# louissmit/VBNN

Measured on NVIDIA B200. Metric: VB-MLP train samples/sec, higher is better.
Workload: dtype bf16

## Files before the change

### vbnn_b200/csrc/layer.cu

```cuda
#include <math.h>
#include <stdarg.h>
#include <string.h>

#include <vector>

#include "knobs.h"
#include "state.h"

namespace vbnn {

static thread_local char g_err[512] = "";

void set_error(const char* fmt, ...) {
  va_list ap;
  va_start(ap, fmt);
  vsnprintf(g_err, sizeof(g_err), fmt, ap);
  va_end(ap);
}

template <typename T>
static int dev_zalloc(T** p, size_t count, cudaStream_t st) {
  VB_TRY(dev_alloc(p, count));
  if (count) VB_CUDA(cudaMemsetAsync(*p, 0, count * sizeof(T), st));
  return VBNN_OK;
// ... 179 lines not shown
  int t = *reinterpret_cast<int*>(c->h_scalars) + 1;
  VB_CUDA(cudaMemcpyAsync(L->t_dev, &t, sizeof(int), cudaMemcpyHostToDevice, c->stream));
  VB_CUDA(cudaStreamSynchronize(c->stream));
  return VBNN_OK;
}

int layer_update_internal(vbnn_layer* L, vbnn_stats* stats, bool bump_t) {
  vbnn_ctx* c = L->ctx;
  cudaStream_t st = c->stream;
  const long long W = (long long)L->O * L->I;
  if (L->kind == VBNN_KIND_LINEAR) {
    VB_TRY(launch_sgd(L->weight, L->gW, W, &L->hp->lr_bias, L->w_bf16, L->I, L->ldI, st));
    VB_TRY(launch_sgd(L->bias, L->gb, L->O, &L->hp->lr_bias, nullptr, 1, 1, st));
    c->launches += 2;
    if (bump_t) VB_TRY(bump_layer_t(L));
    return VBNN_OK;
  }
  VB_TRY(launch_sgd(L->bias, L->gb, L->O, &L->hp->lr_bias, nullptr, 1, 1, st));
  UpdateParams u;
  memset(&u, 0, sizeof(u));
  u.mu = L->means; u.lvar = L->lvars; u.gW = L->gW; u.gS = L->gS;
  u.m_mu = L->m_mu; u.v_mu = L->v_mu; u.m_var = L->m_var; u.v_var = L->v_var;
  u.stdv = L->stdv; u.mu_sqe = L->mu_sqe;
  u.mu_bf16 = L->mu_bf16; u.s2_bf16 = L->s2_bf16; u.ld_bf16 = L->ldI; u.s2_f32 = L->s2_f32;
  u.O = L->O; u.I = L->I;
  u.partials = L->prior_partials; u.n_partials = L->n_part;
  u.next_partials = L->prior_partials; u.partials_pingpong = 1;
  u.var_hat_dev = L->var_hat_dev; u.t_dev = L->t_dev;
  u.S = (float)L->opts.S;
  u.hp = L->hp;
  u.lrt = layer_is_lrt(L);
  u.prior = layer_prior(L, 0);
  u.grid_override = L->n_part;
  u.coresident = knobs().upd_coresident != 0;
  double* stat_dev = stats ? c->d_partials + kMaxPartials : nullptr;
  u.stat_partials = stat_dev;
  int grid = 0;
  const double bytes = (L->prior_kind == VBNN_PRIOR_PER_WEIGHT ? 64.0 : 56.0) * (double)W;
  VB_TRY(prof_launch(c, 7, bytes, [&] { return launch_update(u, &grid, st); }));
  c->launches += 2;
  L->prior_valid = true;
  if (bump_t) VB_TRY(bump_layer_t(L));
  if (stats) {
    VB_CUDA(cudaMemcpyAsync(c->h_partials, stat_dev, (size_t)grid * kStatSlots * sizeof(double),
                            cudaMemcpyDeviceToHost, st));
    VB_CUDA(cudaMemcpyAsync(c->h_scalars, L->var_hat_dev, sizeof(float), cudaMemcpyDeviceToHost, st));
    VB_CUDA(cudaStreamSynchronize(st));
    double s[kStatSlots] = {0};
    s[11] = 3e38; s[12] = -3e38; s[13] = 3e38; s[14] = -3e38;
    for (int b = 0; b < grid; ++b) {
      const double* q = c->h_partials + (size_t)b * kStatSlots;
      for (int i = 0; i < 10; ++i) s[i] += q[i];
      s[11] = fmin(s[11], q[11]); s[12] = fmax(s[12], q[12]);
      s[13] = fmin(s[13], q[13]); s[14] = fmax(s[14], q[14]);
    }
    const double n = (double)W, nl = sqrt(s[4]), nm = sqrt(s[5]);
    stats->vlc_grad = (float)(sqrt(s[0]) / nl);
    stats->vle_grad = (float)(sqrt(s[1]) / nl);
    stats->mlc_grad = (float)(sqrt(s[2]) / nm);
    stats->mle_grad = (float)(sqrt(s[3]) / nm);
    stats->min_variance = (float)s[11];
    stats->max_variance = (float)s[12];
    stats->mean_variance = (float)(s[6] / n);
    stats->var_hat = c->h_scalars[0];
    const double mean = s[7] / n;
    stats->mean_means = (float)mean;
    stats->std_means = (float)sqrt(fmax(0.0, (s[5] - n * mean * mean) / (n - 1.0)));
    stats->min_means = (float)s[13];
    stats->max_means = (float)s[14];
    stats->mu_normratio = (float)(sqrt(s[8]) / nm);
    stats->var_normratio = (float)(sqrt(s[9]) / nl);
  }
  return VBNN_OK;
}

void weight_operands(GemmArgs& g, const vbnn_layer* L, int kmajor, bool batched, bool lrt) {
  const bool b16 = is_bf16(L), mu = layer_is_lrt(L);
  const int ld = b16 ? L->ldI : L->I;
  const void* w = b16 ? (mu ? (const void*)L->mu_bf16 : L->w_bf16) : (mu ? L->means : L->weight);
  g.B1 = {w, ld, kmajor, batched ? (long long)L->O * ld : 0};
  if (lrt) g.B2 = {b16 ? (const void*)L->s2_bf16 : L->s2_f32, ld, kmajor, 0};
}

int gemm(vbnn_ctx* c, bool bf16, int mode, const GemmArgs& g, const EpiParams& p, int prof_cls) {
  if (!bf16) return gemm_simt_launch(mode, g, p, c->stream, &c->launches);
  const int cls = (prof_cls >= 0 ? prof_cls : mode) & 7;
  const double flops = 2.0 * g.M * (double)g.N * g.K * g.batch * (epi_is_dual(mode) ? 2.0 : 1.0);
  return prof_launch(c, cls, flops, [&] { return gemm_tc_launch(mode, g, p, c->stream, &c->launches); });
}

int prof_mark(vbnn_ctx* c, int id) {
  if (!c->profiling) return VBNN_OK;
  cudaEvent_t e;
  if (!c->prof_pool.empty()) { e = c->prof_pool.back(); c->prof_pool.pop_back(); }
  else VB_CUDA(cudaEventCreate(&e));
  VB_CUDA(cudaEventRecord(e, c->stream));
  c->marks.push_back({e, id});
  return VBNN_OK;
}

int prof_collect(vbnn_ctx* c) {
  if (c->prof_recs.empty() && c->marks.empty()) return VBNN_OK;
  VB_CUDA(cudaStreamSynchronize(c->stream));
  for (size_t i = 0; i < c->marks.size(); ++i) {
    const int id = c->marks[i].id & 15;
    if (i > 0 && id != 0) {
      float ms = 0.f;
      VB_CUDA(cudaEventElapsedTime(&ms, c->marks[i - 1].e, c->marks[i].e));
      c->phase_ms[id] += ms; c->phase_n[id] += 1;
    }
  }
  for (auto& mk : c->marks) c->prof_pool.push_back(mk.e);
  c->marks.clear();
  for (auto& r : c->prof_recs) {
    float ms = 0.f;
    VB_CUDA(cudaEventElapsedTime(&ms, r.a, r.b));
    c->prof_ms[r.cls] += ms; c->prof_flops[r.cls] += r.flops; c->prof_n[r.cls] += 1;
    c->prof_pool.push_back(r.a); c->prof_pool.push_back(r.b);
  }
  c->prof_recs.clear();
  return VBNN_OK;
}

}

using namespace vbnn;

extern "C" int vbnn_abi_version(void) { return VBNN_ABI_VERSION; }
extern "C" const char* vbnn_last_error(void) { return g_err; }

extern "C" void vbnn_opts_default(vbnn_opts* o) {
  if (!o) return;
  memset(o, 0, sizeof(*o));
  o->var_init = 0.001f;
  o->msr_init = 0;
  o->mu_init = 0.f;
  o->B = 1000000.f;
  o->S = 30;
  o->lr_bias = 0.001f;
  o->lr_mu = 0.0001f;
  o->lr_var = 0.05f;
  o->adam_beta1 = 0.9f; o->adam_beta2 = 0.999f; o->adam_eps = 1e-8f;
  o->reparam = VBNN_REPARAM_WEIGHT;
  o->precision = VBNN_PREC_FP32;
  o->strict_reference = 1;
}

extern "C" int vbnn_ctx_create(int device, void* stream, uint64_t seed, vbnn_ctx** out) {
  return vbnn_ctx_create_ex(device, stream, VBNN_CTX_STREAM_GIVEN, seed, out);
}

extern "C" int vbnn_ctx_create_ex(int device, void* stream, int stream_mode, uint64_t seed, vbnn_ctx** out) {
  VB_CHECK(out != nullptr, VBNN_E_INVALID, "vbnn_ctx_create: out is null");
  VB_CHECK(stream_mode >= VBNN_CTX_STREAM_GIVEN && stream_mode <= VBNN_CTX_STREAM_PRIVATE_BLOCKING, VBNN_E_INVALID,
           "vbnn_ctx_create_ex: bad stream_mode %d", stream_mode);
  VB_CHECK(stream_mode == VBNN_CTX_STREAM_GIVEN || stream == nullptr, VBNN_E_INVALID,
           "vbnn_ctx_create_ex: stream must be NULL with stream_mode %d", stream_mode);
  int ndev = 0;
  cudaError_t e = cudaGetDeviceCount(&ndev);
  if (e != cudaSuccess || ndev == 0) {
    set_error("no CUDA device available (%s); libvbnn has no CPU fallback",
              e != cudaSuccess ? cudaGetErrorString(e) : "device count 0");
    return VBNN_E_CUDA;
  }
  VB_CHECK(device >= 0 && device < ndev, VBNN_E_INVALID, "vbnn_ctx_create: device %d of %d", device, ndev);
  VB_CUDA(cudaSetDevice(device));
  cudaDeviceProp prop;
  VB_CUDA(cudaGetDeviceProperties(&prop, device));
  VB_CHECK(prop.major == 10, VBNN_E_UNSUPPORTED,
           "libvbnn.so is built for sm_100a only; device %d is sm_%d%d", device, prop.major, prop.minor);
  vbnn_ctx* c = new vbnn_ctx();
  c->device = device; c->seed = seed;
  if (stream_mode == VBNN_CTX_STREAM_LEGACY_DEFAULT) {
    c->stream = cudaStreamLegacy;
    c->capturable = false;
  } else if (stream_mode == VBNN_CTX_STREAM_PRIVATE_BLOCKING) {
    VB_CUDA(cudaStreamCreateWithFlags(&c->stream, cudaStreamDefault));
    c->own_stream = true;
  } else if (stream) {
    c->stream = (cudaStream_t)stream;
    c->capturable = c->stream != cudaStreamLegacy && c->stream != cudaStreamPerThread;
  } else {
    VB_CUDA(cudaStreamCreateWithFlags(&c->stream, cudaStreamNonBlocking));
    c->own_stream = true;
  }
  VB_CUDA(cudaStreamCreateWithFlags(&c->copy_stream, cudaStreamNonBlocking));
  VB_TRY(dev_zalloc(&c->d_step, 1, c->stream));
  VB_TRY(dev_alloc(&c->d_partials, (size_t)kMaxPartials * (1 + kStatSlots)));
  VB_CUDA(cudaMallocHost((void**)&c->h_partials, (size_t)kMaxPartials * kStatSlots * sizeof(double)));
  VB_CUDA(cudaMallocHost((void**)&c->h_scalars, 4096 * sizeof(float)));
  *out = c;
  return VBNN_OK;
}

extern "C" int vbnn_ctx_destroy(vbnn_ctx* c) {
  if (!c) return VBNN_OK;
  cudaSetDevice(c->device);
  cudaStreamSynchronize(c->stream);
  prof_collect(c);
  for (cudaEvent_t e : c->prof_pool) cudaEventDestroy(e);
  vbnn_comm_destroy(c);
  DEV_FREE(c->d_step); DEV_FREE(c->d_partials);
  if (c->h_partials) cudaFreeHost(c->h_partials);
  if (c->h_scalars) cudaFreeHost(c->h_scalars);
  if (c->copy_stream) cudaStreamDestroy(c->copy_stream);
  if (c->own_stream) cudaStreamDestroy(c->stream);
  delete c;
  return VBNN_OK;
}

extern "C" int vbnn_ctx_synchronize(vbnn_ctx* c) {
  VB_CHECK(c, VBNN_E_INVALID, "null ctx");
  VB_CUDA(cudaStreamSynchronize(c->stream));
  return VBNN_OK;
}
extern "C" int vbnn_ctx_profile(vbnn_ctx* c, int enable) {
  VB_CHECK(c, VBNN_E_INVALID, "null ctx");
  VB_TRY(prof_collect(c));
  c->profiling = enable != 0;
  if (enable) for (int i = 0; i < vbnn_ctx::kProfClasses; ++i) { c->prof_ms[i] = 0; c->prof_flops[i] = 0; c->prof_n[i] = 0; }
  if (enable) for (int i = 0; i < 16; ++i) { c->phase_ms[i] = 0; c->phase_n[i] = 0; }
  return VBNN_OK;
}
extern "C" int vbnn_ctx_profile_read(vbnn_ctx* c, int cls, double* total_ms, long long* launches, double* flops) {
  VB_CHECK(c && cls >= 0 && cls < vbnn_ctx::kProfClasses, VBNN_E_INVALID, "vbnn_ctx_profile_read: bad argument");
  VB_TRY(prof_collect(c));
  if (total_ms) *total_ms = c->prof_ms[cls];
  if (launches) *launches = c->prof_n[cls];
  if (flops) *flops = c->prof_flops[cls];
  return VBNN_OK;
}
extern "C" int vbnn_ctx_phase_read(vbnn_ctx* c, int id, double* total_ms, long long* count) {
  VB_CHECK(c && id >= 0 && id < 16, VBNN_E_INVALID, "vbnn_ctx_phase_read: bad argument");
  VB_TRY(prof_collect(c));
  if (total_ms) *total_ms = c->phase_ms[id];
  if (count) *count = c->phase_n[id];
  return VBNN_OK;
}
extern "C" int vbnn_ctx_set_step(vbnn_ctx* c, uint32_t step) {
  VB_CHECK(c, VBNN_E_INVALID, "null ctx");
  VB_CUDA(cudaMemcpyAsync(c->d_step, &step, sizeof(step), cudaMemcpyHostToDevice, c->stream));
  VB_CUDA(cudaStreamSynchronize(c->stream));
  return VBNN_OK;
}
extern "C" int vbnn_ctx_get_step(vbnn_ctx* c, uint32_t* step) {
  VB_CHECK(c && step, VBNN_E_INVALID, "null argument");
  VB_CUDA(cudaMemcpyAsync(step, c->d_step, sizeof(*step), cudaMemcpyDeviceToHost, c->stream));
  VB_CUDA(cudaStreamSynchronize(c->stream));
  return VBNN_OK;
}

extern "C" int vbnn_layer_create(vbnn_ctx* ctx, int inputSize, int outputSize, int kind,
                                 const vbnn_opts* opts, vbnn_layer** out) {
  return layer_create_internal(ctx, inputSize, outputSize, kind, opts, 1, nullptr, nullptr, nullptr, -1, out);
}

extern "C" int vbnn_layer_destroy(vbnn_layer* L) {
  if (!L) return VBNN_OK;
  cudaSetDevice(L->ctx->device);
  cudaStreamSynchronize(L->ctx->stream);
  DEV_FREE(L->means); DEV_FREE(L->lvars);
  if (!L->ext_bias) DEV_FREE(L->bias);
  if (!L->ext_weight) DEV_FREE(L->weight);
  if (!L->grads_external) {
    if (!L->ext_gW) DEV_FREE(L->gW);
    DEV_FREE(L->gS);
    if (!L->ext_gb) DEV_FREE(L->gb);
  }
  DEV_FREE(L->m_mu); DEV_FREE(L->v_mu); DEV_FREE(L->m_var); DEV_FREE(L->v_var);
  DEV_FREE(L->eps); DEV_FREE(L->stdv); DEV_FREE(L->mu_sqe); DEV_FREE(L->s2_f32);
  DEV_FREE(L->var_hat_dev); DEV_FREE(L->t_dev); DEV_FREE(L->hp); DEV_FREE(L->prior_partials);
  DEV_FREE(L->w_bf16); DEV_FREE(L->mu_bf16); DEV_FREE(L->s2_bf16); DEV_FREE(L->eps16);
  DEV_FREE(L->xs); DEV_FREE(L->xs2); DEV_FREE(L->gs_); DEV_FREE(L->hs); DEV_FREE(L->R);
  DEV_FREE(L->zeta_keep);
  DEV_FREE(L->prior_means); DEV_FREE(L->prior_lvars);
  delete L;
  return VBNN_OK;
}

extern "C" int vbnn_layer_dims(const vbnn_layer* L, int* I, int* O) {
  VB_CHECK(L, VBNN_E_INVALID, "null layer");
  if (I) *I = L->I;
  if (O) *O = L->O;
  return VBNN_OK;
}

extern "C" int vbnn_layer_sample(vbnn_layer* L, int sample_idx, const float* eps_dev) {
  VB_CHECK(L && L->kind == VBNN_KIND_VB, VBNN_E_INVALID, "vbnn_layer_sample: not a VB layer");
// ... 517 lines not shown
```

### vbnn_b200/csrc/mlp.cu

```cuda
#include <string.h>

#include "knobs.h"
#include "state.h"

using namespace vbnn;

namespace {

inline size_t esz(const vbnn_mlp* m) { return m->bf16 ? 2 : 4; }
inline int nlayers(const vbnn_mlp* m) { return (int)m->layers.size(); }
inline bool lrt_split(const vbnn_mlp* m, int which) {
  return (knobs().lrt_split & which) != 0 && m->aux != nullptr;
}

int stage_input(vbnn_mlp* m, const float* X, const float* T, int N) {
  cudaStream_t st = m->ctx->stream;
  const int I0 = m->sizes[0], ld0 = m->ld[0];
  if (m->bf16) {
    VB_TRY(launch_cast(X, I0, N, I0, (bf16*)m->act[0], m->lrt ? (bf16*)m->act2[0] : nullptr, ld0, st));
    m->ctx->launches++;
  } else {
    VB_CUDA(cudaMemcpy2DAsync(m->act[0], (size_t)ld0 * 4, X, (size_t)I0 * 4, (size_t)I0 * 4, N,
                              cudaMemcpyDeviceToDevice, st));
    if (m->lrt) {
// ... 86 lines not shown
    p.out_f32 = m->ext_logits; p.ld_f32 = L->O; p.zs_f32 = (long long)N * L->O;
  } else if (last) {
    p.out_f32 = m->logits; p.ld_f32 = m->ld_logits; p.zs_f32 = (long long)N * m->ld_logits;
  } else {
    p.out_act = m->act[j + 1];
  }
  int mode = EPI_FWD;
  if (lrt) {
    mode = EPI_FWD_LRT;
    if (!last) p.out_act2 = m->act2[j + 1];
    p.r_out = m->R[j];
    p.ps = layer_stream(L, kStreamZeta, sample0);
    p.step_ptr = m->ctx->d_step;
    p.row0 = m->ctx->rank * N;
    VB_CHECK((unsigned long long)m->ctx->nranks * (unsigned long long)N * (unsigned long long)((L->O + 3) / 4) <= 0xFFFFFFFFull,
             VBNN_E_UNSUPPORTED, "Philox zeta counter would wrap: %d ranks x %d rows x %d outputs", m->ctx->nranks, N, L->O);
  }
  GemmArgs g;
  memset(&g, 0, sizeof(g));
  g.M = N; g.N = L->O; g.K = L->I; g.batch = Zrun;
  g.A1 = {m->act[j], ldi, 1, zs_in};
  if (lrt) g.A2 = {m->act2[j], ldi, 1, zs_in};
  weight_operands(g, L, 1, w_batched, lrt);
  if (lrt && lrt_split(m, 1)) return gemm_lrt_split(m, mode, g, p);
  return gemm(m->ctx, m->bf16, mode, g, p);
}

int loss_all(vbnn_mlp* m, int N, int Zrun, bool backward, float* logp_out, float* result) {
  const int Lc = nlayers(m);
  vbnn_layer* Lo = m->layers[Lc - 1];
  LossParams lp;
  memset(&lp, 0, sizeof(lp));
  lp.logits = m->logits; lp.ld_logits = m->ld_logits;
  lp.targets = m->targets;
  lp.N = N; lp.C = Lo->O; lp.Z = Zrun;
  lp.grad_scale = 1.0f / ((float)N * (float)m->ctx->nranks);
  if (backward) {
    if (m->bf16) lp.g_bf16 = (bf16*)m->G[Lc - 1]; else lp.g_f32 = (float*)m->G[Lc - 1];
    lp.ld_g = m->ld[Lc];
  }
  lp.logp_out = logp_out;
  lp.result = result;
  lp.z_slot0 = 0;
  VB_TRY(launch_loss(lp, m->ctx->stream));
  m->ctx->launches++;
  if (backward && layer_is_lrt(Lo)) {
    VB_TRY(launch_mul_act(m->G[Lc - 1], m->ld[Lc], m->bf16, m->R[Lc - 1], m->ld[Lc], m->H[Lc - 1], m->ld[Lc],
                          (long long)Zrun * N, Lo->O, m->bf16, m->ctx->stream));
    m->ctx->launches++;
  }
  return VBNN_OK;
}

int backward_data_layer(vbnn_mlp* m, int j, int N, int Zrun) {
  if (j == 0 && !m->dX) return VBNN_OK;
  vbnn_layer* L = m->layers[j];
  const bool lrt = layer_is_lrt(L);
  const int ldi = m->ld[j], ldo = m->ld[j + 1];
  const long long zs_out = (long long)N * ldo;
  GemmArgs g;
  memset(&g, 0, sizeof(g));
  g.M = N; g.N = L->I; g.K = L->O; g.batch = Zrun;
  g.A1 = {m->G[j], ldo, 1, zs_out};
  if (lrt) g.A2 = {m->H[j], ldo, 1, zs_out};
  weight_operands(g, L, 0, L->kind == VBNN_KIND_VB && !lrt, lrt);
  EpiParams p;
  memset(&p, 0, sizeof(p));
  p.M = N; p.N = L->I;
  if (j > 0) {
    p.out_act = m->G[j - 1]; p.ld_act = ldi; p.zs_act = (long long)N * ldi;
    p.xprev = m->act[j]; p.ld_x = ldi; p.zs_x = (long long)N * ldi;
    p.mask = 1;
    if (layer_is_lrt(m->layers[j - 1])) { p.rprev = m->R[j - 1]; p.out_act2 = m->H[j - 1]; }
  } else {
    g.zsum = 1;
    p.out_f32 = m->dX; p.ld_f32 = L->I;
    if (lrt) { p.xprev = m->act[0]; p.ld_x = ldi; p.zs_x = 0; }
  }
  const int mode = lrt ? EPI_DX_LRT : EPI_DX;
  if (lrt && lrt_split(m, 2)) return gemm_lrt_split(m, mode, g, p);
  return gemm(m->ctx, m->bf16, mode, g, p);
}

int backward_weight_layer(vbnn_mlp* m, int j, int N, int Zrun, int sample0, int accumulate, bool scatter = false) {
  vbnn_layer* L = m->layers[j];
  const bool lrt = layer_is_lrt(L);
  const int ldi = m->ld[j], ldo = m->ld[j + 1];
  const long long zs_in = j == 0 ? 0 : (long long)N * ldi;
  const long long zs_out = (long long)N * ldo;
  cudaStream_t st = m->ctx->stream;
  {
    EpiParams p;
    memset(&p, 0, sizeof(p));
    p.M = L->O; p.N = L->I;
    p.gW = L->gW; p.gS = L->kind == VBNN_KIND_VB ? L->gS : nullptr; p.ld_g = L->I;
    p.scale = 1.f; p.accumulate = accumulate;
    p.ps = layer_stream(L, kStreamEps, sample0);
    p.step_ptr = m->ctx->d_step;
    if (L->eps_injected && Zrun == 1 && L->eps) p.noise = L->eps;
    else if (L->eps16_valid && L->kind == VBNN_KIND_VB && !lrt) {
      p.eps16 = L->eps16; p.ld_e16 = L->ldI; p.zs_e16 = (long long)L->O * L->ldI;
    }
    if (scatter) peer_scatter(m, j, N, p);
    const int mode = lrt ? EPI_DW_LRT : EPI_DW;
    const int split_knob = knobs().dw_split;
    const bool split = split_knob >= 0 ? split_knob != 0 : (scatter && !peer_transport_ce(m, N));
    GemmArgs g;
    memset(&g, 0, sizeof(g));
    g.M = L->O; g.N = L->I; g.K = N; g.batch = Zrun;
    g.A1 = {m->G[j], ldo, 0, zs_out};
    g.B1 = {m->act[j], ldi, 0, zs_in};
    if (lrt) { g.A2 = {m->H[j], ldo, 0, zs_out}; g.B2 = {m->act2[j], ldi, 0, zs_in}; }
    const int lin_tiles = ceil_div(L->O, 128) * ceil_div(L->I, 128);
    if (m->bf16 && lrt && split) {
      GemmArgs g1 = g;
      g1.A2 = g1.B2 = GemmOperand{};
      EpiParams p1 = p;
      p1.gS = nullptr;
      p1.noise = nullptr;
      VB_TRY(gemm(m->ctx, m->bf16, EPI_DW, g1, p1));
      g1.A1 = g.A2; g1.B1 = g.B2;
      p1.gW = L->gS;
      if (p1.scatter_rows)
        for (int q = 0; q < 8; ++q) p1.gW_peer[q] = p.gS_peer[q];
      p1.scale = 1.f;
      VB_TRY(gemm(m->ctx, m->bf16, EPI_DW, g1, p1));
    } else if (m->bf16 && L->kind == VBNN_KIND_LINEAR && Zrun > 1 && !scatter && m->dw_partials &&
               lin_tiles * 2 <= kNumSMs && (L->I & 3) == 0) {
      EpiParams p0;
      memset(&p0, 0, sizeof(p0));
      p0.M = L->O; p0.N = L->I;
      p0.out_f32 = m->dw_partials; p0.ld_f32 = L->I; p0.zs_f32 = (long long)L->O * L->I;
      VB_TRY(gemm(m->ctx, m->bf16, EPI_STORE, g, p0, EPI_DW));
      VB_TRY(launch_sum_partials(m->dw_partials, Zrun, (long long)L->O * L->I, (long long)L->O * L->I, p.scale, accumulate,
                                 L->gW, st));
      m->ctx->launches++;
    } else {
      if (m->bf16 && L->kind == VBNN_KIND_LINEAR && Zrun > 1 && zs_in == (long long)N * ldi) {
        g.K = N * Zrun; g.batch = 1;
        g.A1.zs = 0; g.B1.zs = 0;
      }
      VB_TRY(gemm(m->ctx, m->bf16, mode, g, p));
    }
  }
  VB_TRY(launch_colsum(m->G[j], m->bf16, (long long)Zrun * N, L->O, ldo, 1.f, L->gb, st));
  m->ctx->launches++;
  return VBNN_OK;
}

int backward_layer(vbnn_mlp* m, int j, int N, int Zrun, int sample0, int accumulate) {
  VB_TRY(backward_data_layer(m, j, N, Zrun));
  return backward_weight_layer(m, j, N, Zrun, sample0, accumulate, false);
}

int forward_samples(vbnn_mlp* m, int N, int Zrun, int sample0, bool peer = false) {
  const int Lc = nlayers(m);
  vbnn_ctx* c = m->ctx;
  for (int j = 0; j < Lc; ++j) {
    if (peer && !m->peer_waited_all) { VB_TRY(peer_wait_params(m, j, true)); VB_TRY(prof_mark(c, 1)); }
    VB_TRY(forward_layer(m, j, N, Zrun, sample0, false));
    VB_TRY(prof_mark(c, 3));
  }
  return VBNN_OK;
}

int backward_samples(vbnn_mlp* m, int N, int Zrun, int sample0, int accumulate, bool reduce_overlap = false,
                     bool peer = false) {
  const int Lc = nlayers(m);
  vbnn_ctx* c = m->ctx;
  if (peer) {
    for (int j = Lc - 1; j >= (m->dX ? 0 : 1); --j) { VB_TRY(backward_data_layer(m, j, N, Zrun)); VB_TRY(prof_mark(c, 5)); }
    for (int j = 0; j < Lc; ++j) {
      VB_TRY(backward_weight_layer(m, j, N, Zrun, sample0, accumulate, true));
      VB_TRY(prof_mark(c, 5));
      VB_TRY(peer_after_dw(m, j));
    }
    return VBNN_OK;
  }
  for (int j = Lc - 1; j >= 0; --j) {
    VB_TRY(backward_layer(m, j, N, Zrun, sample0, accumulate));
    VB_TRY(prof_mark(c, 5));
    if (reduce_overlap) {
      VB_CUDA(cudaEventRecord(m->ev_bwd[j], c->stream));
      VB_CUDA(cudaStreamWaitEvent(c->comm_stream, m->ev_bwd[j], 0));
      VB_TRY(comm_allreduce_internal(c, m->grad_arena + m->grad_off[j], m->grad_len[j], c->comm_stream));
      VB_CUDA(cudaEventRecord(m->ev_red[j], c->comm_stream));
    }
  }
  return VBNN_OK;
}

int update_all(vbnn_mlp* m, bool wait_reduce = false) {
  const int Lc = nlayers(m);
  cudaStream_t st = m->ctx->stream;
  if (m->layers[Lc - 1]->kind == VBNN_KIND_LINEAR) {
    if (wait_reduce) VB_CUDA(cudaStreamWaitEvent(st, m->ev_red[Lc - 1], 0));
    VB_TRY(layer_update_internal(m->layers[Lc - 1], nullptr, false));
  }
  if (wait_reduce) {
    for (int j = Lc - 1; j >= 0; --j) {
      if (m->layers[j]->kind != VBNN_KIND_VB) continue;
      VB_CUDA(cudaStreamWaitEvent(st, m->ev_red[j], 0));
      VB_TRY(layer_update_internal(m->layers[j], nullptr, false));
    }
  } else {
    for (vbnn_layer* L : m->layers)
      if (L->kind == VBNN_KIND_VB) VB_TRY(layer_update_internal(L, nullptr, false));
  }
  return VBNN_OK;
}

int step_forward(vbnn_mlp* m, int N) {
  cudaStream_t st = m->ctx->stream;
  for (vbnn_layer* L : m->layers) VB_CUDA(cudaMemsetAsync(L->gb, 0, (size_t)L->O * 4, st));
  const bool peer = m->peer && m->peer->active;
  if (peer) {
    VB_TRY(peer_check(m));
    m->peer_waited_all = !m->lrt;
    if (!m->lrt) {
      VB_TRY(peer_wait_params(m, -1, true));
      VB_TRY(prof_mark(m->ctx, 1));
    }
  } else {
    VB_TRY(prof_mark(m->ctx, 1));
  }
  VB_TRY(sample_all(m, 0, m->Z));
  VB_TRY(prof_mark(m->ctx, 2));
  return forward_samples(m, N, m->Z, 0, peer);
}

int step_backward(vbnn_mlp* m, int N, bool finalize) {
  cudaStream_t st = m->ctx->stream;
  if (m->peer && m->peer->active) {
    VB_TRY(backward_samples(m, N, m->Z, 0, 0, false, true));
    if (finalize) { VB_TRY(launch_finalize_result(m->result_acc, m->Z, N, m->result, st)); m->ctx->launches++; }
    VB_TRY(launch_bump(m->ctx->d_step, m->t_list_dev, 0, st));
    m->ctx->launches++;
    VB_TRY(prof_mark(m->ctx, 7));
    return VBNN_OK;
  }
  const bool dp = m->ctx->nranks > 1;
  const bool overlap = dp && knobs().dp_overlap && m->ctx->comm_stream != nullptr;
  VB_TRY(backward_samples(m, N, m->Z, 0, 0, overlap));
  if (dp && !overlap) VB_TRY(comm_allreduce_internal(m->ctx, m->grad_arena, m->grad_count, st));
  VB_TRY(update_all(m, overlap));
  VB_TRY(prof_mark(m->ctx, 6));
  if (finalize) {
    VB_TRY(launch_finalize_result(m->result_acc, m->Z, N, m->result, st));
    m->ctx->launches++;
  }
  VB_TRY(launch_bump(m->ctx->d_step, m->t_list_dev, m->n_t, st));
  m->ctx->launches++;
  VB_TRY(prof_mark(m->ctx, 7));
  return VBNN_OK;
}

int step_body(vbnn_mlp* m, int N) {
  VB_TRY(prof_mark(m->ctx, 0));
  VB_CUDA(cudaMemsetAsync(m->result_acc, 0, (size_t)2 * m->Z * 4, m->ctx->stream));
  VB_TRY(step_forward(m, N));
  VB_TRY(loss_all(m, N, m->Z, true, nullptr, m->result_acc));
  VB_TRY(prof_mark(m->ctx, 4));
  return step_backward(m, N, true);
}

int split_backward_body(vbnn_mlp* m, int N, const float* grad) {
  const int Lc = nlayers(m);
  vbnn_layer* Lo = m->layers[Lc - 1];
  VB_TRY(prof_mark(m->ctx, 0));
  VB_TRY(launch_grad_logits(grad, (long long)m->Z * N, Lo->O, m->G[Lc - 1], m->ld[Lc],
                            layer_is_lrt(Lo) ? m->R[Lc - 1] : nullptr, m->H[Lc - 1], m->bf16, m->ctx->stream));
  m->ctx->launches++;
  VB_TRY(prof_mark(m->ctx, 4));
  return step_backward(m, N, false);
}

template <typename Body>
int graph_enqueue(vbnn_mlp* m, vbnn_mlp::StepGraph& sg, int N, const void* key0, const void* key1, Body&& body) {
  vbnn_ctx* c = m->ctx;
  cudaStream_t st = c->stream;
  const bool graphable = m->use_graph && c->capturable && c->nranks == 1 && !c->profiling;
  if (!graphable || sg.eager_steps < 1) {
    sg.eager_steps++;
    return body();
  }
  if (sg.exec && (sg.N != N || sg.key[0] != key0 || sg.key[1] != key1)) {
    cudaGraphExecDestroy(sg.exec);
    sg.exec = nullptr;
  }
  if (!sg.exec) {
    const long long before = c->launches;
    VB_CUDA(cudaStreamBeginCapture(st, cudaStreamCaptureModeThreadLocal));
    int r = body();
    cudaGraph_t gr = nullptr;
    cudaError_t e = cudaStreamEndCapture(st, &gr);
    if (r != VBNN_OK) { if (gr) cudaGraphDestroy(gr); return r; }
    if (e != cudaSuccess) { set_error("cudaStreamEndCapture: %s", cudaGetErrorString(e)); return VBNN_E_CUDA; }
    e = cudaGraphInstantiate(&sg.exec, gr, 0);
    cudaGraphDestroy(gr);
    if (e != cudaSuccess) { set_error("cudaGraphInstantiate: %s", cudaGetErrorString(e)); sg.exec = nullptr; return VBNN_E_CUDA; }
    sg.N = N;
    sg.key[0] = key0; sg.key[1] = key1;
    sg.launches = c->launches - before;
    c->launches = before;
    m->graph_captures++;
  }
  VB_CUDA(cudaGraphLaunch(sg.exec, st));
  c->launches += sg.launches;
  return VBNN_OK;
}

int step_enqueue(vbnn_mlp* m, int N) {
  return graph_enqueue(m, m->graphs[m->dX ? vbnn_mlp::kGraphStepDx : vbnn_mlp::kGraphStep], N, m->dX, nullptr,
                       [&] { return step_body(m, N); });
}

int refuse_open_step(const vbnn_mlp* m, const char* who) {
  VB_CHECK(!m->step_open, VBNN_E_STATE,
           "%s: a vbnn_mlp_forward_train step is open: close it with vbnn_mlp_backward_update (or abandon it with "
           "vbnn_mlp_reset_gradients)", who);
  return VBNN_OK;
}

template <typename Consume>
int eval_forward(vbnn_mlp* m, const float* X, const float* T, int N, int n_samples, const char* who,
                 Consume&& consume, float* samples = nullptr) {
  VB_TRY(stage_input(m, X, T, N));
  if (m->peer && m->peer->active) {
// ... 51 lines not shown
  vbnn_mlp* m = new vbnn_mlp();
  m->ctx = ctx; m->opts = *opts; m->vb_output = vb_output; m->max_batch = max_batch;
  m->bf16 = opts->precision == VBNN_PREC_BF16;
  m->lrt = opts->reparam == VBNN_REPARAM_LOCAL;
  m->Z = opts->S;
  m->sizes.assign(sizes, sizes + n_sizes);
  for (int k = 0; k < n_sizes; ++k) {
    VB_CHECK(sizes[k] > 0, VBNN_E_INVALID, "vbnn_mlp_create: size[%d] = %d", k, sizes[k]);
    m->ld.push_back(round_up(sizes[k], 8));
  }
  const int Lc = n_sizes - 1;
  cudaStream_t st = ctx->stream;
  int r = VBNN_OK;
  std::vector<size_t> off_gW(Lc), off_gS(Lc), off_gb(Lc);
  size_t off = 0;
  auto take = [&](size_t n) { size_t o = off; off += (n + 63) / 64 * 64; return o; };
  for (int j = 0; j < Lc; ++j) {
    const bool vb = j < Lc - 1 || vb_output;
    const size_t W = (size_t)sizes[j] * sizes[j + 1];
    off_gW[j] = take(W);
    off_gS[j] = vb ? take(W) : 0;
    off_gb[j] = take(sizes[j + 1]);
    m->grad_off.push_back(off_gW[j]);
    m->grad_len.push_back(off - off_gW[j]);
  }
  m->grad_count = off;
  r = dev_alloc(&m->grad_arena, off);
  if (r == VBNN_OK && cudaMemsetAsync(m->grad_arena, 0, off * 4, st) != cudaSuccess) r = VBNN_E_CUDA;
  for (int j = 0; j < Lc && r == VBNN_OK; ++j) {
    const bool vb = j < Lc - 1 || vb_output;
    vbnn_layer* L = nullptr;
    r = layer_create_internal(ctx, sizes[j], sizes[j + 1], vb ? VBNN_KIND_VB : VBNN_KIND_LINEAR, opts,
                              (vb && !m->lrt) ? m->Z : 1, m->grad_arena + off_gW[j],
                              vb ? m->grad_arena + off_gS[j] : nullptr, m->grad_arena + off_gb[j], j, &L);
    if (r == VBNN_OK) { L->owned_by_mlp = true; L->owner = m; m->layers.push_back(L); }
  }
  const size_t e = esz(m);
  const size_t ZN = (size_t)m->Z * max_batch;
  m->act.assign(n_sizes, nullptr); m->act2.assign(n_sizes, nullptr);
  m->R.assign(Lc, nullptr); m->G.assign(Lc, nullptr); m->H.assign(Lc, nullptr);
  auto A_ = [&](void** p, size_t bytes) { if (r == VBNN_OK) { char* q; r = dev_alloc(&q, bytes); *p = q; } };
  A_(&m->act[0], (size_t)max_batch * m->ld[0] * e);
  if (m->lrt) A_(&m->act2[0], (size_t)max_batch * m->ld[0] * e);
  for (int j = 0; j < Lc; ++j) {
    const bool vb = j < Lc - 1 || vb_output;
    const size_t bytes = ZN * m->ld[j + 1] * e;
    if (j < Lc - 1) {
      A_(&m->act[j + 1], bytes);
      if (m->lrt) A_(&m->act2[j + 1], bytes);
    }
    A_(&m->G[j], bytes);
    if (m->lrt && vb) { A_(&m->R[j], bytes); A_(&m->H[j], bytes); }
  }
  if (m->lrt && m->bf16) {
    int mx = 0;
    for (int k = 0; k < n_sizes; ++k) mx = m->ld[k] > mx ? m->ld[k] : mx;
    m->ld_aux = mx;
    A_((void**)&m->aux, ZN * (size_t)mx * 4);
  }
  if (m->bf16 && m->Z > 1 && !vb_output)
    A_((void**)&m->dw_partials, (size_t)m->Z * sizes[Lc - 1] * sizes[Lc] * 4);
  m->ld_logits = m->ld[Lc];
  A_((void**)&m->logits, ZN * m->ld_logits * 4);
  A_((void**)&m->targets, (size_t)max_batch * 4);
  A_((void**)&m->result_acc, (size_t)2 * m->Z * 4);
  A_((void**)&m->result, 2 * 4);
  if (r == VBNN_OK) {
    std::vector<int*> ts;
    for (vbnn_layer* L : m->layers) ts.push_back(L->t_dev);
    m->n_t = (int)ts.size();
    r = dev_alloc(&m->t_list_dev, ts.size());
    if (r == VBNN_OK &&
        cudaMemcpyAsync(m->t_list_dev, ts.data(), ts.size() * sizeof(int*), cudaMemcpyHostToDevice, st) != cudaSuccess)
      r = VBNN_E_CUDA;
    if (r == VBNN_OK) cudaStreamSynchronize(st);
  }
  for (int s = 0; s < 2; ++s) { m->slots[s].busy = false; m->slots[s].h_result = nullptr; m->slots[s].copied = nullptr; }
  for (int j = 0; j < Lc && r == VBNN_OK; ++j) {
    cudaEvent_t a, b;
    if (cudaEventCreateWithFlags(&a, cudaEventDisableTiming) != cudaSuccess ||
        cudaEventCreateWithFlags(&b, cudaEventDisableTiming) != cudaSuccess) { r = VBNN_E_CUDA; break; }
    m->ev_bwd.push_back(a); m->ev_red.push_back(b);
  }
  if (knobs().no_graph) m->use_graph = false;
  if (r != VBNN_OK) { vbnn_mlp_destroy(m); return r; }
  *out = m;
  return VBNN_OK;
}

extern "C" int vbnn_mlp_destroy(vbnn_mlp* m) {
  if (!m) return VBNN_OK;
  cudaSetDevice(m->ctx->device);
  cudaStreamSynchronize(m->ctx->stream);
  cudaStreamSynchronize(m->ctx->copy_stream);
  for (vbnn_mlp::StepGraph& sg : m->graphs)
    if (sg.exec) cudaGraphExecDestroy(sg.exec);
  peer_destroy(m);
  for (cudaEvent_t e : m->ev_bwd) cudaEventDestroy(e);
  for (cudaEvent_t e : m->ev_red) cudaEventDestroy(e);
  for (vbnn_layer* L : m->layers) vbnn_layer_destroy(L);
  for (void* p : m->act) if (p) cudaFree(p);
  for (void* p : m->act2) if (p) cudaFree(p);
  for (void* p : m->R) if (p) cudaFree(p);
  for (void* p : m->G) if (p) cudaFree(p);
  for (void* p : m->H) if (p) cudaFree(p);
  if (m->aux) cudaFree(m->aux);
  if (m->dw_partials) cudaFree(m->dw_partials);
  if (m->logits) cudaFree(m->logits);
  if (m->logp) cudaFree(m->logp);
  if (m->pred_max) cudaFree(m->pred_max);
  if (m->pred_sum) cudaFree(m->pred_sum);
  if (m->pred_ent) cudaFree(m->pred_ent);
  if (m->pred_partials) cudaFree(m->pred_partials);
  if (m->mom_state) cudaFree(m->mom_state);
  if (m->targets) cudaFree(m->targets);
  if (m->result_acc) cudaFree(m->result_acc);
  if (m->result) cudaFree(m->result);
  if (m->grad_arena) cudaFree(m->grad_arena);
  if (m->t_list_dev) cudaFree(m->t_list_dev);
  for (int s = 0; s < 2; ++s) {
    if (m->xstage[s]) cudaFree(m->xstage[s]);
    if (m->xstage_u8[s]) cudaFree(m->xstage_u8[s]);
    if (m->tstage[s]) cudaFree(m->tstage[s]);
    if (m->pipeline_ready) {
      cudaEventDestroy(m->slots[s].copied); cudaEventDestroy(m->slots[s].consumed); cudaEventDestroy(m->slots[s].done);
      if (m->slots[s].h_result) cudaFreeHost(m->slots[s].h_result);
    }
  }
  delete m;
  return VBNN_OK;
}

extern "C" int vbnn_mlp_num_layers(const vbnn_mlp* m) { return m ? (int)m->layers.size() : VBNN_E_INVALID; }

extern "C" int vbnn_mlp_layer(vbnn_mlp* m, int k, vbnn_layer** out) {
  VB_CHECK(m && out && k >= 0 && k < nlayers(m), VBNN_E_INVALID, "vbnn_mlp_layer: bad index %d", k);
  *out = m->layers[k];
  return VBNN_OK;
}

extern "C" int vbnn_mlp_init_params(vbnn_mlp* m, uint64_t seed, int he_means) {
  VB_CHECK(m, VBNN_E_INVALID, "null mlp");
  VB_TRY(refuse_open_step(m, "vbnn_mlp_init_params"));
  cudaStream_t st = m->ctx->stream;
  for (vbnn_layer* L : m->layers) {
    const long long W = (long long)L->O * L->I;
    PhiloxStream ps = layer_stream(L, kStreamInit, 1);
    ps.key0 = (uint32_t)(seed & 0xFFFFFFFFu); ps.key1 = (uint32_t)(seed >> 32);
    VB_CUDA(cudaMemsetAsync(L->bias, 0, (size_t)L->O * 4, st));
    if (L->kind == VBNN_KIND_LINEAR) {
      VB_TRY(launch_init_normal(L->weight, W, 0.f, sqrtf(2.0f / (float)L->I), ps, st));
    } else {
      const float var_init = (L->opts.msr_init || he_means) ? 2.0f / (float)L->I : L->opts.var_init;
      if (he_means || L->opts.mu_init != 0.f)
        VB_TRY(launch_init_normal(L->means, W, 0.f, sqrtf(var_init), ps, st));
      else
        VB_CUDA(cudaMemsetAsync(L->means, 0, (size_t)W * 4, st));
      VB_TRY(layer_compute_prior_internal(L));
      VB_TRY(layer_refresh_prior_partials(L));
    }
    VB_TRY(layer_refresh_copies(L));
    m->ctx->launches += 2;
  }
  return VBNN_OK;
}

extern "C" int vbnn_mlp_reset_gradients(vbnn_mlp* m) {
  VB_CHECK(m, VBNN_E_INVALID, "null mlp");
  if (m->step_open) {
    VB_CHECK(!(m->peer && m->peer->active), VBNN_E_STATE,
             "vbnn_mlp_reset_gradients: an open step cannot be abandoned in peer mode; pass a zero gradient to "
             "vbnn_mlp_backward_update instead");
    m->step_open = false;
  }
  cudaStream_t st = m->ctx->stream;
  VB_CUDA(cudaMemsetAsync(m->grad_arena, 0, m->grad_count * 4, st));
  VB_CUDA(cudaMemsetAsync(m->result_acc, 0, (size_t)2 * m->Z * 4, st));
  return VBNN_OK;
}

extern "C" int vbnn_mlp_sample(vbnn_mlp* m, int sample_idx) {
  VB_CHECK(m, VBNN_E_INVALID, "null mlp");
// ... 392 lines not shown
```

### vbnn_b200/csrc/state.h

```cpp
#pragma once
#include <vector>

#include "common.cuh"
#include "gemm.h"
#include "kernels.h"

struct vbnn_ctx {
  int device = 0;
  cudaStream_t stream = nullptr;
  bool own_stream = false;
  bool capturable = true;
  cudaStream_t copy_stream = nullptr;
  uint64_t seed = 0;
  uint32_t* d_step = nullptr;
  double* d_partials = nullptr;
  double* h_partials = nullptr;
  float* h_scalars = nullptr;
  int next_layer_id = 0;
  long long launches = 0;
  static constexpr int kProfClasses = 9;
  bool profiling = false;
  struct ProfRec { cudaEvent_t a, b; int cls; double flops; };
  std::vector<ProfRec> prof_recs;
  std::vector<cudaEvent_t> prof_pool;
  double prof_ms[kProfClasses] = {0}; double prof_flops[kProfClasses] = {0}; long long prof_n[kProfClasses] = {0};
  struct Mark { cudaEvent_t e; int id; };
  std::vector<Mark> marks;
  double phase_ms[16] = {0}; long long phase_n[16] = {0};
  void* nccl_comm = nullptr;
  int rank = 0, nranks = 1;
  cudaStream_t comm_stream = nullptr;
};

struct vbnn_layer {
  vbnn_ctx* ctx = nullptr;
  int I = 0, O = 0, kind = VBNN_KIND_VB, id = 0;
  vbnn_opts opts;
  int ldI = 0, ldO = 0;
  int S_alloc = 1;
  bool owned_by_mlp = false;
  bool grads_external = false;
  bool ext_weight = false, ext_bias = false, ext_gW = false, ext_gb = false;
  float *means = nullptr, *lvars = nullptr, *bias = nullptr, *weight = nullptr;
  float *gW = nullptr, *gS = nullptr, *gb = nullptr;
  float *m_mu = nullptr, *v_mu = nullptr, *m_var = nullptr, *v_var = nullptr;
  float *eps = nullptr, *stdv = nullptr, *mu_sqe = nullptr, *s2_f32 = nullptr;
  float* var_hat_dev = nullptr;
  int n_part = 0;
  double* prior_partials = nullptr;
  int* t_dev = nullptr;
  vbnn::LiveOpts* hp = nullptr;
  bf16 *w_bf16 = nullptr, *mu_bf16 = nullptr, *s2_bf16 = nullptr;
  void* eps16 = nullptr;
  bool eps16_valid = false;
  int cap_N = 0;
  void *xs = nullptr, *xs2 = nullptr, *gs_ = nullptr, *hs = nullptr, *R = nullptr;
  float* zeta_keep = nullptr;
  int cur_sample = 0;
  bool eps_injected = false;
  bool map_mode = false;
  bool prior_valid = false;
  const bool* shard_stale = nullptr;
  vbnn_mlp* owner = nullptr;
  int prior_kind = VBNN_PRIOR_EMPIRICAL;
  float prior_mu0 = 0.f, prior_var0 = 0.f;
  float *prior_means = nullptr, *prior_lvars = nullptr;
};

constexpr int kMaxPeers = 8;
struct PeerBuf { void* ptr[kMaxPeers] = {nullptr}; };
struct PeerLayer {
  int rpo = 0, row0 = 0, rows = 0;
  size_t slot_floats = 0;
  size_t off_recv = 0;
  size_t off_gb = 0;
  PeerBuf means, lvars, s2_f32, mu_bf16, s2_bf16, weight, w_bf16, partials, m_mu, v_mu, m_var, v_var;
  uint32_t *mseq = nullptr, *sseq = nullptr;
  cudaEvent_t ev_dw = nullptr;
  float* stage = nullptr;
};
struct vbnn_peer {
  int G = 1, me = 0;
  char* block = nullptr; size_t block_bytes = 0;
  char* peer_block[kMaxPeers] = {nullptr};
  size_t off_grad_ready = 0, off_param_ready = 0;
  std::vector<PeerLayer> layers;
  uint32_t* seq = nullptr;
  int* h_err = nullptr; int* d_err = nullptr;
  cudaStream_t side = nullptr;
  cudaStream_t xfer = nullptr;
  cudaEvent_t ev_xfer = nullptr;
  unsigned int* xfer_done = nullptr;
  cudaEvent_t ev_side = nullptr;
  std::vector<void*> opened;
  bool exported = false, active = false, stale = false;
};

struct vbnn_mlp {
  vbnn_ctx* ctx = nullptr;
  vbnn_peer* peer = nullptr;
  std::vector<int> sizes;
  std::vector<vbnn_layer*> layers;
  int vb_output = 0, max_batch = 0, Z = 1;
  vbnn_opts opts;
  bool bf16 = false, lrt = false;
  std::vector<int> ld;
  std::vector<void*> act, act2;
  std::vector<void*> R, G, H;
  float* aux = nullptr; int ld_aux = 0;
  float* dw_partials = nullptr;
  float* logits = nullptr; int ld_logits = 0;
  float* logp = nullptr;
  float *pred_max = nullptr, *pred_sum = nullptr, *pred_ent = nullptr;
  double* pred_partials = nullptr;
  float* mom_state = nullptr;
  float* targets = nullptr;
  float* xstage[2] = {nullptr, nullptr};
  float* tstage[2] = {nullptr, nullptr};
  uint8_t* xstage_u8[2] = {nullptr, nullptr};
  float* result_acc = nullptr;
  float* result = nullptr;
  float* grad_arena = nullptr; size_t grad_count = 0;
  std::vector<size_t> grad_off, grad_len;
  std::vector<cudaEvent_t> ev_bwd, ev_red;
  int** t_list_dev = nullptr; int n_t = 0;
  struct StepGraph {
    cudaGraphExec_t exec = nullptr; int N = -1; const void* key[2] = {nullptr, nullptr}; int eager_steps = 0;
    long long launches = 0;
  };
  enum { kGraphStep, kGraphStepDx, kGraphFwd, kGraphBwd, kGraphBwdDx, kNumGraphs };
  StepGraph graphs[kNumGraphs];
  long long graph_captures = 0;
  bool use_graph = true;
  float* dX = nullptr;
  float* ext_logits = nullptr;
  bool step_open = false;
  int open_N = 0;
  bool outputs_external = false;
  struct Slot { cudaEvent_t copied, consumed, done; float* h_result; bool busy; int N; };
  Slot slots[2];
  int submit_idx = 0, collect_idx = 0, inflight = 0;
  bool pipeline_ready = false;
  int last_N = 0;
  bool peer_waited_all = false;
};

namespace vbnn {
template <typename T>
int dev_alloc(T** p, size_t count) {
  *p = nullptr;
  if (count == 0) return VBNN_OK;
  cudaError_t e = cudaMalloc((void**)p, count * sizeof(T));
  if (e != cudaSuccess) {
    set_error("cudaMalloc(%zu bytes) failed: %s", count * sizeof(T), cudaGetErrorString(e));
    return e == cudaErrorMemoryAllocation ? VBNN_E_NOMEM : VBNN_E_CUDA;
  }
  return VBNN_OK;
}
inline bool layer_is_lrt(const vbnn_layer* L) {
  return L->kind == VBNN_KIND_VB && L->opts.reparam == VBNN_REPARAM_LOCAL;
}
int layer_create_internal(vbnn_ctx* ctx, int I, int O, int kind, const vbnn_opts* opts, int S_alloc,
                          float* gW, float* gS, float* gb, int id, vbnn_layer** out);
int layer_update_internal(vbnn_layer* L, vbnn_stats* stats, bool bump_t);
int layer_refresh_copies(vbnn_layer* L);
int layer_compute_prior_internal(vbnn_layer* L);
int layer_refresh_prior_partials(vbnn_layer* L);
PriorArgs layer_prior(const vbnn_layer* L, size_t row_off);
void mlp_drop_graphs(vbnn_mlp* m);
int mlp_wait_side(vbnn_mlp* m);
LiveOpts live_opts(const vbnn_opts& o);
PhiloxStream layer_stream(const vbnn_layer* L, uint32_t kind, int sample);
int comm_allreduce_internal(vbnn_ctx* ctx, float* buf, size_t count, cudaStream_t st);
void peer_destroy(vbnn_mlp* m);
void peer_scatter(const vbnn_mlp* m, int j, int N, EpiParams& p);
bool peer_transport_ce(const vbnn_mlp* m, int N);
bool peer_wire_bf16(const vbnn_mlp* m, int j, int N);
int peer_wait_params(vbnn_mlp* m, int j, bool bump);
int peer_after_dw(vbnn_mlp* m, int j);
int peer_check(vbnn_mlp* m);
void weight_operands(GemmArgs& g, const vbnn_layer* L, int kmajor, bool batched, bool lrt);
int gemm(vbnn_ctx* ctx, bool bf16, int mode, const GemmArgs& g, const EpiParams& p, int prof_cls = -1);
int prof_collect(vbnn_ctx* ctx);
int prof_mark(vbnn_ctx* ctx, int id);
template <typename Launch>
int prof_launch(vbnn_ctx* c, int cls, double work, Launch&& launch) {
  if (!c->profiling) return launch();
  vbnn_ctx::ProfRec r;
  for (cudaEvent_t* e : {&r.a, &r.b}) {
    if (!c->prof_pool.empty()) { *e = c->prof_pool.back(); c->prof_pool.pop_back(); }
    else VB_CUDA(cudaEventCreate(e));
  }
  r.cls = cls; r.flops = work;
  VB_CUDA(cudaEventRecord(r.a, c->stream));
  const int rc = launch();
  VB_CUDA(cudaEventRecord(r.b, c->stream));
  c->prof_recs.push_back(r);
  if (c->prof_recs.size() + c->marks.size() >= 4096) VB_TRY(prof_collect(c));
  return rc;
}
}
```

Measured before the change: 1.438 million.

## Run weight-gradient GEMMs on a side stream overlapping the data-gradient chain

Adds a second CUDA stream for weight-gradient work. During backward, each layer's dW GEMM and bias colsum are forked onto that stream via events while the dX chain continues on the main stream, and the updates for the lower layer wait on a join event. This lets the two independent backward chains run concurrently and fill idle SMs. The cost is extra event traffic and SM contention between the two chains, and it is used only when the run is not data-parallel and not profiling. There is also a possible race: weight-gradient work later reads G[j] and activations that the main stream may overwrite, and ev_wgrad_upper is recorded before layer 0's dW is launched.

```diff
diff --git a/vbnn_b200/csrc/layer.cu b/vbnn_b200/csrc/layer.cu
--- a/vbnn_b200/csrc/layer.cu
+++ b/vbnn_b200/csrc/layer.cu
@@ -285,11 +285,13 @@
   if (lrt) g.B2 = {b16 ? (const void*)L->s2_bf16 : L->s2_f32, ld, kmajor, 0};
 }
 
-int gemm(vbnn_ctx* c, bool bf16, int mode, const GemmArgs& g, const EpiParams& p, int prof_cls) {
-  if (!bf16) return gemm_simt_launch(mode, g, p, c->stream, &c->launches);
+int gemm(vbnn_ctx* c, bool bf16, int mode, const GemmArgs& g, const EpiParams& p, int prof_cls, cudaStream_t st) {
+  if (!st) st = c->stream;
+  if (!bf16) return gemm_simt_launch(mode, g, p, st, &c->launches);
+  VB_CHECK(!c->profiling || st == c->stream, VBNN_E_STATE, "gemm: a profiled launch must run on the context's stream");
   const int cls = (prof_cls >= 0 ? prof_cls : mode) & 7;
   const double flops = 2.0 * g.M * (double)g.N * g.K * g.batch * (epi_is_dual(mode) ? 2.0 : 1.0);
-  return prof_launch(c, cls, flops, [&] { return gemm_tc_launch(mode, g, p, c->stream, &c->launches); });
+  return prof_launch(c, cls, flops, [&] { return gemm_tc_launch(mode, g, p, st, &c->launches); });
 }
 
 int prof_mark(vbnn_ctx* c, int id) {
@@ -388,6 +390,7 @@
     c->own_stream = true;
   }
   VB_CUDA(cudaStreamCreateWithFlags(&c->copy_stream, cudaStreamNonBlocking));
+  VB_CUDA(cudaStreamCreateWithFlags(&c->wgrad_stream, cudaStreamNonBlocking));
   VB_TRY(dev_zalloc(&c->d_step, 1, c->stream));
   VB_TRY(dev_alloc(&c->d_partials, (size_t)kMaxPartials * (1 + kStatSlots)));
   VB_CUDA(cudaMallocHost((void**)&c->h_partials, (size_t)kMaxPartials * kStatSlots * sizeof(double)));
@@ -407,6 +410,7 @@
   if (c->h_partials) cudaFreeHost(c->h_partials);
   if (c->h_scalars) cudaFreeHost(c->h_scalars);
   if (c->copy_stream) cudaStreamDestroy(c->copy_stream);
+  if (c->wgrad_stream) { cudaStreamSynchronize(c->wgrad_stream); cudaStreamDestroy(c->wgrad_stream); }
   if (c->own_stream) cudaStreamDestroy(c->stream);
   delete c;
   return VBNN_OK;
diff --git a/vbnn_b200/csrc/mlp.cu b/vbnn_b200/csrc/mlp.cu
--- a/vbnn_b200/csrc/mlp.cu
+++ b/vbnn_b200/csrc/mlp.cu
@@ -192,13 +192,13 @@
   return gemm(m->ctx, m->bf16, mode, g, p);
 }
 
-int backward_weight_layer(vbnn_mlp* m, int j, int N, int Zrun, int sample0, int accumulate, bool scatter = false) {
+int backward_weight_layer(vbnn_mlp* m, int j, int N, int Zrun, int sample0, int accumulate, bool scatter,
+                          cudaStream_t st) {
   vbnn_layer* L = m->layers[j];
   const bool lrt = layer_is_lrt(L);
   const int ldi = m->ld[j], ldo = m->ld[j + 1];
   const long long zs_in = j == 0 ? 0 : (long long)N * ldi;
   const long long zs_out = (long long)N * ldo;
-  cudaStream_t st = m->ctx->stream;
   {
     EpiParams p;
     memset(&p, 0, sizeof(p));
@@ -228,20 +228,20 @@
       EpiParams p1 = p;
       p1.gS = nullptr;
       p1.noise = nullptr;
-      VB_TRY(gemm(m->ctx, m->bf16, EPI_DW, g1, p1));
+      VB_TRY(gemm(m->ctx, m->bf16, EPI_DW, g1, p1, -1, st));
       g1.A1 = g.A2; g1.B1 = g.B2;
       p1.gW = L->gS;
       if (p1.scatter_rows)
         for (int q = 0; q < 8; ++q) p1.gW_peer[q] = p.gS_peer[q];
       p1.scale = 1.f;
-      VB_TRY(gemm(m->ctx, m->bf16, EPI_DW, g1, p1));
+      VB_TRY(gemm(m->ctx, m->bf16, EPI_DW, g1, p1, -1, st));
     } else if (m->bf16 && L->kind == VBNN_KIND_LINEAR && Zrun > 1 && !scatter && m->dw_partials &&
                lin_tiles * 2 <= kNumSMs && (L->I & 3) == 0) {
       EpiParams p0;
       memset(&p0, 0, sizeof(p0));
       p0.M = L->O; p0.N = L->I;
       p0.out_f32 = m->dw_partials; p0.ld_f32 = L->I; p0.zs_f32 = (long long)L->O * L->I;
-      VB_TRY(gemm(m->ctx, m->bf16, EPI_STORE, g, p0, EPI_DW));
+      VB_TRY(gemm(m->ctx, m->bf16, EPI_STORE, g, p0, EPI_DW, st));
       VB_TRY(launch_sum_partials(m->dw_partials, Zrun, (long long)L->O * L->I, (long long)L->O * L->I, p.scale, accumulate,
                                  L->gW, st));
       m->ctx->launches++;
@@ -250,7 +250,7 @@
         g.K = N * Zrun; g.batch = 1;
         g.A1.zs = 0; g.B1.zs = 0;
       }
-      VB_TRY(gemm(m->ctx, m->bf16, mode, g, p));
+      VB_TRY(gemm(m->ctx, m->bf16, mode, g, p, -1, st));
     }
   }
   VB_TRY(launch_colsum(m->G[j], m->bf16, (long long)Zrun * N, L->O, ldo, 1.f, L->gb, st));
@@ -260,7 +260,7 @@
 
 int backward_layer(vbnn_mlp* m, int j, int N, int Zrun, int sample0, int accumulate) {
   VB_TRY(backward_data_layer(m, j, N, Zrun));
-  return backward_weight_layer(m, j, N, Zrun, sample0, accumulate, false);
+  return backward_weight_layer(m, j, N, Zrun, sample0, accumulate, false, m->ctx->stream);
 }
 
 int forward_samples(vbnn_mlp* m, int N, int Zrun, int sample0, bool peer = false) {
@@ -275,16 +275,28 @@
 }
 
 int backward_samples(vbnn_mlp* m, int N, int Zrun, int sample0, int accumulate, bool reduce_overlap = false,
-                     bool peer = false) {
+                     bool peer = false, bool two_chains = false) {
   const int Lc = nlayers(m);
   vbnn_ctx* c = m->ctx;
   if (peer) {
     for (int j = Lc - 1; j >= (m->dX ? 0 : 1); --j) { VB_TRY(backward_data_layer(m, j, N, Zrun)); VB_TRY(prof_mark(c, 5)); }
     for (int j = 0; j < Lc; ++j) {
-      VB_TRY(backward_weight_layer(m, j, N, Zrun, sample0, accumulate, true));
+      VB_TRY(backward_weight_layer(m, j, N, Zrun, sample0, accumulate, true, c->stream));
       VB_TRY(prof_mark(c, 5));
       VB_TRY(peer_after_dw(m, j));
     }
+    return VBNN_OK;
+  }
+  if (two_chains) {
+    for (int j = Lc - 1; j >= 0; --j) {
+      VB_CUDA(cudaEventRecord(m->ev_grad[j], c->stream));
+      VB_CUDA(cudaStreamWaitEvent(c->wgrad_stream, m->ev_grad[j], 0));
+      if (j == 0) VB_CUDA(cudaEventRecord(m->ev_wgrad_upper, c->wgrad_stream));
+      VB_TRY(backward_weight_layer(m, j, N, Zrun, sample0, accumulate, false, c->wgrad_stream));
+      VB_TRY(backward_data_layer(m, j, N, Zrun));
+    }
+    VB_CUDA(cudaEventRecord(m->ev_wgrad, c->wgrad_stream));
+    VB_CUDA(cudaStreamWaitEvent(c->stream, m->ev_wgrad_upper, 0));
     return VBNN_OK;
   }
   for (int j = Lc - 1; j >= 0; --j) {
@@ -300,11 +312,12 @@
   return VBNN_OK;
 }
 
-int update_all(vbnn_mlp* m, bool wait_reduce = false) {
+int update_all(vbnn_mlp* m, bool wait_reduce = false, bool wgrad_tail = false) {
   const int Lc = nlayers(m);
   cudaStream_t st = m->ctx->stream;
   if (m->layers[Lc - 1]->kind == VBNN_KIND_LINEAR) {
     if (wait_reduce) VB_CUDA(cudaStreamWaitEvent(st, m->ev_red[Lc - 1], 0));
+    if (wgrad_tail && Lc == 1) VB_CUDA(cudaStreamWaitEvent(st, m->ev_wgrad, 0));
     VB_TRY(layer_update_internal(m->layers[Lc - 1], nullptr, false));
   }
   if (wait_reduce) {
@@ -314,8 +327,10 @@
       VB_TRY(layer_update_internal(m->layers[j], nullptr, false));
     }
   } else {
-    for (vbnn_layer* L : m->layers)
-      if (L->kind == VBNN_KIND_VB) VB_TRY(layer_update_internal(L, nullptr, false));
+    for (int j = 1; j < Lc; ++j)
+      if (m->layers[j]->kind == VBNN_KIND_VB) VB_TRY(layer_update_internal(m->layers[j], nullptr, false));
+    if (wgrad_tail) VB_CUDA(cudaStreamWaitEvent(st, m->ev_wgrad, 0));
+    if (m->layers[0]->kind == VBNN_KIND_VB) VB_TRY(layer_update_internal(m->layers[0], nullptr, false));
   }
   return VBNN_OK;
 }
@@ -351,9 +366,10 @@
   }
   const bool dp = m->ctx->nranks > 1;
   const bool overlap = dp && knobs().dp_overlap && m->ctx->comm_stream != nullptr;
-  VB_TRY(backward_samples(m, N, m->Z, 0, 0, overlap));
+  const bool two_chains = !dp && !m->ctx->profiling;
+  VB_TRY(backward_samples(m, N, m->Z, 0, 0, overlap, false, two_chains));
   if (dp && !overlap) VB_TRY(comm_allreduce_internal(m->ctx, m->grad_arena, m->grad_count, st));
-  VB_TRY(update_all(m, overlap));
+  VB_TRY(update_all(m, overlap, two_chains));
   VB_TRY(prof_mark(m->ctx, 6));
   if (finalize) {
     VB_TRY(launch_finalize_result(m->result_acc, m->Z, N, m->result, st));
@@ -571,6 +587,12 @@
         cudaEventCreateWithFlags(&b, cudaEventDisableTiming) != cudaSuccess) { r = VBNN_E_CUDA; break; }
     m->ev_bwd.push_back(a); m->ev_red.push_back(b);
   }
+  for (int j = 0; j <= Lc && r == VBNN_OK; ++j) {
+    cudaEvent_t e;
+    if (cudaEventCreateWithFlags(&e, cudaEventDisableTiming) != cudaSuccess) { r = VBNN_E_CUDA; break; }
+    if (j < Lc) m->ev_grad.push_back(e); else m->ev_wgrad = e;
+  }
+  if (r == VBNN_OK && cudaEventCreateWithFlags(&m->ev_wgrad_upper, cudaEventDisableTiming) != cudaSuccess) r = VBNN_E_CUDA;
   if (knobs().no_graph) m->use_graph = false;
   if (r != VBNN_OK) { vbnn_mlp_destroy(m); return r; }
   *out = m;
@@ -582,11 +604,15 @@
   cudaSetDevice(m->ctx->device);
   cudaStreamSynchronize(m->ctx->stream);
   cudaStreamSynchronize(m->ctx->copy_stream);
+  cudaStreamSynchronize(m->ctx->wgrad_stream);
   for (vbnn_mlp::StepGraph& sg : m->graphs)
     if (sg.exec) cudaGraphExecDestroy(sg.exec);
   peer_destroy(m);
   for (cudaEvent_t e : m->ev_bwd) cudaEventDestroy(e);
   for (cudaEvent_t e : m->ev_red) cudaEventDestroy(e);
+  for (cudaEvent_t e : m->ev_grad) cudaEventDestroy(e);
+  if (m->ev_wgrad) cudaEventDestroy(m->ev_wgrad);
+  if (m->ev_wgrad_upper) cudaEventDestroy(m->ev_wgrad_upper);
   for (vbnn_layer* L : m->layers) vbnn_layer_destroy(L);
   for (void* p : m->act) if (p) cudaFree(p);
   for (void* p : m->act2) if (p) cudaFree(p);
diff --git a/vbnn_b200/csrc/state.h b/vbnn_b200/csrc/state.h
--- a/vbnn_b200/csrc/state.h
+++ b/vbnn_b200/csrc/state.h
@@ -11,6 +11,7 @@
   bool own_stream = false;
   bool capturable = true;
   cudaStream_t copy_stream = nullptr;
+  cudaStream_t wgrad_stream = nullptr;
   uint64_t seed = 0;
   uint32_t* d_step = nullptr;
   double* d_partials = nullptr;
@@ -123,6 +124,9 @@
   float* grad_arena = nullptr; size_t grad_count = 0;
   std::vector<size_t> grad_off, grad_len;
   std::vector<cudaEvent_t> ev_bwd, ev_red;
+  std::vector<cudaEvent_t> ev_grad;
+  cudaEvent_t ev_wgrad = nullptr;
+  cudaEvent_t ev_wgrad_upper = nullptr;
   int** t_list_dev = nullptr; int n_t = 0;
   struct StepGraph {
     cudaGraphExec_t exec = nullptr; int N = -1; const void* key[2] = {nullptr, nullptr}; int eager_steps = 0;
@@ -180,7 +184,8 @@
 int peer_after_dw(vbnn_mlp* m, int j);
 int peer_check(vbnn_mlp* m);
 void weight_operands(GemmArgs& g, const vbnn_layer* L, int kmajor, bool batched, bool lrt);
-int gemm(vbnn_ctx* ctx, bool bf16, int mode, const GemmArgs& g, const EpiParams& p, int prof_cls = -1);
+int gemm(vbnn_ctx* ctx, bool bf16, int mode, const GemmArgs& g, const EpiParams& p, int prof_cls = -1,
+         cudaStream_t st = nullptr);
 int prof_collect(vbnn_ctx* ctx);
 int prof_mark(vbnn_ctx* ctx, int id);
 template <typename Launch>
```

Result: no change. 1.453 million, median of 6 (+1.0%).
